# maraxen/trex

Measured on AMD Instinct MI355X. Metric: site-node-state updates/sec (Sankoff fwd+grad), higher is better.
Workload: dtype f32; 1 GPU; C4: 1024 random 32-taxa topologies x 5000 sites x 4 states, softmin tau=0.5 fwd (DP table written) + grad, split over 1 GPU(s) (1024 trees on rank 0); trees=1024, trees_rank0=1024, taxa=32, sites=5000, states=4, hipgraph=True, parallelism=tree-batch x1, settle_steps=35

## Files before the change

trex_amd/csrc/plan.cpp:

```cpp
#include <algorithm>
#include <cstdlib>
#include <cstdint>
#include <cstring>
#include <functional>
#include <queue>
#include <set>
#include <vector>

#include "trex_common.h"

namespace trex {

namespace {

constexpr int kKindSent = 0, kKindLeaf = 1, kKindInt = 2;

struct Child {
  int kind;
  int index;
};

bool plan_one_tree(const int32_t* ch, int n_all, int32_t* fwd, int32_t* bt,
                   int* n_slots, int* bt_ok, int* n_dag, int* n_unreached) {
  const int nl = (n_all + 1) / 2;
  const int ni = n_all - nl;
  std::vector<Child> kids(2 * ni);
  std::vector<int> refs(ni, 0);
  for (int r = 0; r < ni; ++r) {
    const int node = nl + r;
    for (int k = 0; k < 2; ++k) {
      const int c = ch[2 * node + k];
      if (c < -1 || c >= n_all) return false;
      Child cd;
      if (c == -1 || c >= node) {
        cd = {kKindSent, 0};
      } else if (c < nl) {
        cd = {kKindLeaf, c};
      } else {
        cd = {kKindInt, c - nl};
        refs[c - nl] += 1;
      }
      kids[2 * r + k] = cd;
    }
  }
  int dag = 0;
  for (int r = 0; r < ni; ++r) dag += refs[r] > 1;
  *n_dag = dag;

  std::vector<int> need(ni, 1);
  for (int r = 0; r < ni; ++r) {
    int a = 0, b = 0;
    for (int k = 0; k < 2; ++k) {
      const Child& cd = kids[2 * r + k];
      if (cd.kind == kKindInt) {
        const int n = need[cd.index];
        if (n > a) { b = a; a = n; } else if (n > b) { b = n; }
      }
    }
    need[r] = std::max({1, a, b + 1});
  }

  std::vector<int> order;
  order.reserve(ni);
  std::vector<char> done(ni, 0);
  auto visit = [&](int start) {
    std::vector<std::pair<int, int>> st;
    st.push_back({start, 0});
    while (!st.empty()) {
      auto [r, ph] = st.back();
      st.pop_back();
      if (done[r]) continue;
      if (ph == 1) {
        done[r] = 1;
        order.push_back(r);
        continue;
// ... 7 lines not shown
      if (light >= 0 && !done[light]) st.push_back({light, 0});
      if (heavy >= 0 && !done[heavy]) st.push_back({heavy, 0});
    }
  };
  for (int r = 0; r < ni - 1; ++r)
    if (refs[r] == 0) visit(r);
  visit(ni - 1);
  if ((int)order.size() != ni) return false;

  std::vector<int> pos(ni, 0), consumer(ni, -1);
  for (int k = 0; k < ni; ++k) pos[order[k]] = k;
  for (int r = 0; r < ni; ++r)
    for (int k = 0; k < 2; ++k)
      if (kids[2 * r + k].kind == kKindInt) consumer[kids[2 * r + k].index] = r;
  std::vector<char> bypass(ni, 0);
  for (int r = 0; r < ni; ++r)
    bypass[r] = refs[r] == 1 && consumer[r] >= 0 && pos[consumer[r]] == pos[r] + 1;

  std::vector<int> remaining(refs), slot(ni, 0xFF);
  std::set<int> free_slots;
  int top = 0, maxs = 0;
  for (int r : order) {
    for (int k = 0; k < 2; ++k) {
      const Child& cd = kids[2 * r + k];
      if (cd.kind != kKindInt || bypass[cd.index]) continue;
      if (--remaining[cd.index] == 0) free_slots.insert(slot[cd.index]);
    }
    if (refs[r] > 0 && !bypass[r]) {
      int s;
      if (!free_slots.empty()) {
        s = *free_slots.begin();
        free_slots.erase(free_slots.begin());
      } else {
        s = top++;
      }
      slot[r] = s;
      maxs = std::max(maxs, s + 1);
    }
  }
  if (maxs > 250) return false;
  *n_slots = maxs;

  std::vector<char> reach(ni, 0);
  reach[ni - 1] = 1;
  for (int r = ni - 1; r >= 0; --r) {
    if (!reach[r]) continue;
    for (int k = 0; k < 2; ++k)
      if (kids[2 * r + k].kind == kKindInt) reach[kids[2 * r + k].index] = 1;
  }
  int unr = 0;
  for (int r = 0; r < ni; ++r) unr += !reach[r];
  *n_unreached = unr;

  static const bool defer_on = [] {
    const char* e = std::getenv("TREX_DEFER");
    return !(e && e[0] == '0');
  }();
  std::vector<char> deferred(ni, 0);
  if (defer_on)
    for (int c = 0; c < ni; ++c)
      deferred[c] = refs[c] == 1 && consumer[c] >= 0 && reach[consumer[c]] &&
                    kids[2 * c].kind != kKindInt && kids[2 * c + 1].kind != kKindInt;

  std::vector<char> seen(ni, 0);
  std::vector<int32_t> enc(4 * ni);
  for (int k = ni - 1; k >= 0; --k) {
    const int r = order[k];
    int32_t* e = &enc[4 * k];
    e[0] = (r & 0xFFFF) | ((slot[r] & 0xFF) << 16);
    for (int j = 0; j < 2; ++j) {
      const Child& cd = kids[2 * r + j];
      int32_t d = (cd.index & 0xFFFF) | (cd.kind << 24);
      if (cd.kind == kKindInt) {
        d |= (slot[cd.index] & 0xFF) << 16;
        if (bypass[cd.index]) d |= kChildPrev;
        if (deferred[cd.index]) d |= kChildDeferred;
        if (reach[r]) {
          if (seen[cd.index]) d |= kStepAccumulate;
          seen[cd.index] = 1;
        }
      }
      e[1 + j] = d;
    }
    int32_t f = 0;
    if (r == ni - 1) f |= kStepRoot;
    if (!reach[r]) f |= kStepUnreached;
    if (bypass[r]) f |= kStepToNext;
    if (deferred[r]) f |= kStepDeferredIn;
    e[3] = f;
  }
  if (order.back() != ni - 1) return false;
  std::memcpy(fwd, enc.data(), enc.size() * sizeof(int32_t));

  std::vector<int> last_parent(ni, -1), last_slot(ni, -1);
  std::vector<char> visited(ni, 0);
  std::vector<std::pair<int, int>> stk;
  stk.push_back({n_all - 1, -1});
  int64_t steps = 0;
  const int64_t cap = 1LL << 22;
  bool ok = true;
  while (!stk.empty()) {
    if (++steps > cap || (int64_t)stk.size() > 4LL * n_all) { ok = false; break; }
    auto [node, from] = stk.back();
    stk.pop_back();
    if (node < nl) continue;
    const int x = node - nl;
    visited[x] = 1;
    if (from >= 0) { last_parent[x] = from >> 1; last_slot[x] = from & 1; }
    const int c0 = ch[2 * node], c1 = ch[2 * node + 1];
    if (c0 == node || c1 == node) { ok = false; break; }
// ... 166 lines not shown
    if (kd == kKindSent) return 0;
    if (kd == kKindLeaf) return (c & 0xFFFF) | (kKindLeaf << 24);
    if (task[c]) return (c & 0xFFFF) | (slot[c] << 16) | (kKindInt << 24);
    const int32_t d0 = desc(c, 0), d1 = desc(c, 1);
    inl[c] = (int)(ient.size() / 4);
    ient.insert(ient.end(), {c, d0, d1, height[c]});
    return (inl[c] & 0xFFFF) | (kKindInline << 24);
  };
  const int n_steps = (int)order.size();
  int32_t* offs = region + 4;
  int32_t* steps = region + lp_steps_offset(ni);
  for (int s = 0; s <= S; ++s) offs[s] = n_steps;
  for (int k = n_steps - 1; k >= 0; --k) offs[stage[order[k]]] = k;
  for (int s = S - 1; s >= 0; --s) offs[s] = std::min(offs[s], offs[s + 1]);
  for (int k = 0; k < n_steps; ++k) {
    const int r = order[k];
    steps[4 * k] = (r & 0xFFFF) | (slot[r] << 16);
    steps[4 * k + 1] = desc(r, 0);
    steps[4 * k + 2] = desc(r, 1);
    steps[4 * k + 3] = r == root ? kStepRoot : 0;
  }
  if (!ient.empty()) std::memcpy(steps + 4LL * n_steps, ient.data(), ient.size() * sizeof(int32_t));
  region[0] = S;
  region[1] = n_slots;
  region[2] = n_steps;
  region[3] = (int)(ient.size() / 4);
  return n_slots;
}

}

}

extern "C" int64_t trex_plan_ints(int B, int n_all) {
  if (B <= 0 || n_all < 2) return 0;
  const int ni = n_all - (n_all + 1) / 2;
  return TREX_PLAN_HEADER_INTS + (int64_t)B * ni * 6 +
         (int64_t)B * (trex::staged_tree_ints(ni) + trex::lp_tree_ints(ni));
}

extern "C" int trex_plan_build(const int32_t* children, int B, int n_all,
                               int32_t* plan, int32_t* info) {
  using namespace trex;
  if (!children || !plan || B <= 0 || n_all < 3 || n_all > 65535)
    return set_error(TREX_E_ARG, "trex_plan_build: bad arguments (B=%d n_all=%d)", B, n_all);
  const int nl = (n_all + 1) / 2;
  const int ni = n_all - nl;
  std::memset(plan, 0, sizeof(int32_t) * TREX_PLAN_HEADER_INTS);
  int32_t* fwd = plan + TREX_PLAN_HEADER_INTS;
  int32_t* bt = fwd + (int64_t)B * ni * 4;
  int32_t* staged = bt + (int64_t)B * ni * 2;
  int32_t* lanes = staged + (int64_t)B * staged_tree_ints(ni);
  int max_slots = 0, all_bt_ok = 1, dag = 0, unr = 0, lp_slots = 0;
  for (int b = 0; b < B; ++b) {
    int s = 0, ok = 0, d = 0, u = 0;
    if (!plan_one_tree(children + (int64_t)b * n_all * 2, n_all, fwd + (int64_t)b * ni * 4,
                       bt + (int64_t)b * ni * 2, &s, &ok, &d, &u))
      return set_error(TREX_E_TOPOLOGY, "trex_plan_build: tree %d has an invalid child list", b);
    stage_one_tree(children + (int64_t)b * n_all * 2, n_all, staged + b * staged_tree_ints(ni));
    const int ls = lane_program_one_tree(children + (int64_t)b * n_all * 2, n_all,
                                         lanes + b * lp_tree_ints(ni));
    lp_slots = (ls < 0 || lp_slots < 0) ? -1 : std::max(lp_slots, ls);
    max_slots = std::max(max_slots, s);
    all_bt_ok &= ok;
    dag += d;
    unr += u;
  }
  plan[0] = kPlanMagic;
  plan[1] = B;
  plan[2] = n_all;
  plan[3] = nl;
  plan[4] = ni;
  plan[5] = max_slots;
  plan[6] = all_bt_ok;
  plan[7] = lp_slots;
  if (info) {
    info[0] = max_slots | ((lp_slots < 0 ? 0 : lp_slots + 1) << 16);
    info[1] = all_bt_ok;
    info[2] = dag;
    info[3] = unr;
  }
  return TREX_OK;
}

namespace trex {
namespace {
constexpr int32_t kRaggedMagic = 0x54525247;
constexpr int kRaggedMetaInts = 12;

bool ragged_shapes(const int32_t* n_all, const int32_t* L, int B, int64_t* steps, int64_t* items) {
  *steps = 0;
  *items = 0;
  for (int b = 0; b < B; ++b) {
    if (n_all[b] < 3 || n_all[b] > 65535 || L[b] <= 0) return false;
    *steps += n_all[b] - (n_all[b] + 1) / 2;
    *items += (L[b] + 63) / 64;
  }
  return *items <= 0x7FFFFFFF;
}
}
}

extern "C" int64_t trex_ragged_plan_ints(int B, const int32_t* n_all, const int32_t* L) {
  if (B <= 0 || !n_all || !L) return 0;
  int64_t steps, items;
  if (!trex::ragged_shapes(n_all, L, B, &steps, &items)) return 0;
  return TREX_PLAN_HEADER_INTS + (int64_t)B * trex::kRaggedMetaInts + items + steps * 6;
}

extern "C" int trex_ragged_plan_build(const int32_t* children, const int32_t* n_all,
                                      const int32_t* L, int B, int32_t* plan, int64_t* info) {
  using namespace trex;
  int64_t steps, items;
  if (!children || !n_all || !L || !plan || B <= 0 || !ragged_shapes(n_all, L, B, &steps, &items))
    return set_error(TREX_E_ARG, "trex_ragged_plan_build: bad arguments (B=%d)", B);
  int32_t* meta = plan + TREX_PLAN_HEADER_INTS;
  int32_t* ritem = meta + (int64_t)B * kRaggedMetaInts;
  int32_t* fwd = ritem + items;
  int32_t* bt = fwd + steps * 4;
  std::memset(plan, 0, sizeof(int32_t) * TREX_PLAN_HEADER_INTS);
  int64_t step_off = 0, item_off = 0, site_off = 0, leaf_off = 0, rows_off = 0, child_off = 0;
  int max_slots = 0, max_nl = 0, max_ni = 0, all_ok = 1, dag = 0, unr = 0;
  for (int b = 0; b < B; ++b) {
    const int na = n_all[b];
    const int nl = (na + 1) / 2;
    const int ni = na - nl;
    int s = 0, ok = 0, d = 0, u = 0;
    if (!plan_one_tree(children + child_off, na, fwd + step_off * 4, bt + step_off * 2, &s, &ok, &d,
                       &u))
      return set_error(TREX_E_TOPOLOGY, "trex_ragged_plan_build: tree %d has an invalid child list",
                       b);
    if (site_off > 0x7FFFFFFF)
      return set_error(TREX_E_UNSUPPORTED, "trex_ragged_plan_build: more than 2^31 sites");
    if ((int64_t)ni * L[b] * 4 * 4 > 0x7FFFFFF0LL)
      return set_error(TREX_E_UNSUPPORTED, "trex_ragged_plan_build: tree %d's DP table exceeds 2 GiB",
                       b);
    int32_t* m = meta + (int64_t)b * kRaggedMetaInts;
    m[0] = (int32_t)step_off;
    m[1] = ni;
    m[2] = nl;
    m[3] = L[b];
    m[4] = (int32_t)site_off;
    m[5] = (int32_t)item_off;
    m[6] = (int32_t)(leaf_off & 0xFFFFFFFF);
    m[7] = (int32_t)(leaf_off >> 32);
    m[8] = (int32_t)(rows_off & 0xFFFFFFFF);
    m[9] = (int32_t)(rows_off >> 32);
    const int tiles = (L[b] + 63) / 64;
    for (int t = 0; t < tiles; ++t) ritem[item_off + t] = b;
    max_slots = std::max(max_slots, s);
    max_nl = std::max(max_nl, nl);
    max_ni = std::max(max_ni, ni);
    all_ok &= ok;
    dag += d;
    unr += u;
    step_off += ni;
    item_off += tiles;
    site_off += L[b];
    leaf_off += (int64_t)nl * L[b];
    rows_off += (int64_t)ni * L[b];
    child_off += 2LL * na;
  }
  plan[0] = kRaggedMagic;
  plan[1] = B;
  plan[2] = (int32_t)steps;
  plan[3] = (int32_t)items;
  plan[4] = max_slots;
  plan[5] = max_nl;
  plan[6] = all_ok;
  plan[7] = max_ni;
  if (info) {
    info[0] = max_slots;
    info[1] = max_nl;
    info[2] = items;
    info[3] = leaf_off;
    info[4] = rows_off;
    info[5] = site_off;
    info[6] = all_ok;
    info[7] = dag + ((int64_t)unr << 32);
  }
  return TREX_OK;
}
// ... 1 lines not shown
```

trex_amd/csrc/sankoff.hip:

```cpp
#include <hip/hip_runtime.h>

#include <algorithm>
#include <cmath>
#include <cstdlib>
#include <cstring>
#include <mutex>
#include <string>

#include "sankoff_dev.h"
#include "trex_common.h"

namespace trex {

namespace {

thread_local char g_err[512] = "no error";


template <int SPT>
__device__ __forceinline__ void ld(const float* __restrict__ p, float (&o)[SPT]) {
  if constexpr (SPT == 4) {
    const float4 v = *reinterpret_cast<const float4*>(p);
    o[0] = v.x; o[1] = v.y; o[2] = v.z; o[3] = v.w;
  } else if constexpr (SPT == 2) {
// ... 301 lines not shown
    for (int i = 0; i < Q; ++i) sv[i] = kdot<Q>(cf.k[i], u);
  }
}

template <int Q, int SPT, int MODE, bool SYM = false>
__device__ __forceinline__ void message(const Coef<Q>& cf, float a, float bcoef,
                                        const float (&d)[Q][SPT], float (&m)[Q][SPT]) {
  if constexpr (MODE == kHard) {
#pragma unroll
    for (int i = 0; i < Q; ++i)
#pragma unroll
      for (int s = 0; s < SPT; ++s) {
        float v = cf.c[i][0] + d[0][s];
#pragma unroll
        for (int j = 1; j < Q; ++j) v = fminf(v, cf.c[i][j] + d[j][s]);
        m[i][s] = v;
      }
  } else if constexpr (MODE == kSoftK) {
#pragma unroll
    for (int s = 0; s < SPT; ++s) {
      float md = d[0][s];
#pragma unroll
      for (int j = 1; j < Q; ++j) md = fminf(md, d[j][s]);
      const float mda = md * a;
      float u[Q];
#pragma unroll
      for (int j = 0; j < Q; ++j) u[j] = fast_exp2(fmaf(-d[j][s], a, mda));
      const float base = md + cf.cmin;
      float sv[Q];
      kvec<Q, SYM>(cf, u, sv);
#pragma unroll
      for (int i = 0; i < Q; ++i) m[i][s] = fmaf(-bcoef, fast_log2(sv[i]), base);
    }
  } else {
#pragma unroll
    for (int i = 0; i < Q; ++i)
#pragma unroll
      for (int s = 0; s < SPT; ++s) {
        float x[Q];
        float mn = INFINITY;
#pragma unroll
        for (int j = 0; j < Q; ++j) {
          x[j] = cf.c[i][j] + d[j][s];
          mn = fminf(mn, x[j]);
        }
        float acc = 0.0f;
#pragma unroll
        for (int j = 0; j < Q; ++j) acc += fast_exp2((mn - x[j]) * a);
        m[i][s] = fmaf(-bcoef, fast_log2(acc), mn);
      }
  }
}

template <int Q, int SPT, int MODE, bool SYM = false>
__device__ __forceinline__ void message_adjoint(const Coef<Q>& cf, float a,
                                                const float (&d)[Q][SPT],
                                                const float (&g)[Q][SPT],
                                                float (&acc)[Q][Q], float (&gc)[Q][SPT]) {
#pragma unroll
  for (int s = 0; s < SPT; ++s) {
    if constexpr (MODE == kHard) {
#pragma unroll
      for (int j = 0; j < Q; ++j) gc[j][s] = 0.0f;
#pragma unroll
      for (int i = 0; i < Q; ++i) {
        float x[Q];
        float mn = cf.c[i][0] + d[0][s];
        x[0] = mn;
#pragma unroll
        for (int j = 1; j < Q; ++j) {
          x[j] = cf.c[i][j] + d[j][s];
          mn = fminf(mn, x[j]);
        }
        float cnt = 0.0f;
#pragma unroll
        for (int j = 0; j < Q; ++j) cnt += (x[j] == mn) ? 1.0f : 0.0f;
        const float r = g[i][s] / cnt;
#pragma unroll
        for (int j = 0; j < Q; ++j) {
          const float w = (x[j] == mn) ? r : 0.0f;
          acc[i][j] += w;
          gc[j][s] += w;
        }
      }
    } else if constexpr (MODE == kSoftK) {
      float md = d[0][s];
#pragma unroll
      for (int j = 1; j < Q; ++j) md = fminf(md, d[j][s]);
      const float mda = md * a;
      float u[Q];
#pragma unroll
      for (int j = 0; j < Q; ++j) u[j] = fast_exp2(fmaf(-d[j][s], a, mda));
      float r[Q];
      float sv[Q];
      kvec<Q, SYM>(cf, u, sv);
#pragma unroll
      for (int i = 0; i < Q; ++i) r[i] = g[i][s] * __builtin_amdgcn_rcpf(sv[i]);
#pragma unroll
      for (int i = 0; i < Q; ++i) axpy<Q>(acc[i], r[i], u);
      float t[Q];
#pragma unroll
      for (int j = 0; j < Q; ++j) t[j] = r[0] * cf.k[0][j];
#pragma unroll
      for (int i = 1; i < Q; ++i) axpy<Q>(t, r[i], cf.k[i]);
#pragma unroll
      for (int j = 0; j < Q; ++j) gc[j][s] = u[j] * t[j];
    } else {
#pragma unroll
      for (int j = 0; j < Q; ++j) gc[j][s] = 0.0f;
#pragma unroll
      for (int i = 0; i < Q; ++i) {
        float x[Q];
        float mn = INFINITY;
#pragma unroll
        for (int j = 0; j < Q; ++j) {
          x[j] = cf.c[i][j] + d[j][s];
          mn = fminf(mn, x[j]);
        }
        float e[Q];
        float sm = 0.0f;
#pragma unroll
        for (int j = 0; j < Q; ++j) {
          e[j] = fast_exp2((mn - x[j]) * a);
          sm += e[j];
        }
        const float r = g[i][s] * __builtin_amdgcn_rcpf(sm);
#pragma unroll
        for (int j = 0; j < Q; ++j) {
          const float w = r * e[j];
          acc[i][j] += w;
          gc[j][s] += w;
        }
      }
    }
  }
}

template <int Q, int SPT, bool SOFT>
__device__ __forceinline__ void root_score(const float (&d)[Q][SPT], float a, float bcoef,
                                           bool hard_root, float (&score)[SPT],
                                           float (&w)[Q][SPT]) {
#pragma unroll
  for (int s = 0; s < SPT; ++s) {
    float mn = d[0][s];
#pragma unroll
    for (int i = 1; i < Q; ++i) mn = fminf(mn, d[i][s]);
    if (!SOFT || hard_root) {
      float cnt = 0.0f;
#pragma unroll
      for (int i = 0; i < Q; ++i) cnt += (d[i][s] == mn) ? 1.0f : 0.0f;
      const float r = 1.0f / cnt;
#pragma unroll
      for (int i = 0; i < Q; ++i) w[i][s] = (d[i][s] == mn) ? r : 0.0f;
      score[s] = mn;
    } else {
      float sm = 0.0f;
#pragma unroll
      for (int i = 0; i < Q; ++i) {
        w[i][s] = fast_exp2((mn - d[i][s]) * a);
        sm += w[i][s];
      }
      const float r = __builtin_amdgcn_rcpf(sm);
#pragma unroll
      for (int i = 0; i < Q; ++i) w[i][s] *= r;
      score[s] = fmaf(-bcoef, fast_log2(sm), mn);
    }
  }
}


struct KArgs {
  const int4* steps;
  const int8_t* leaves;
  const float* cost;
  int n_int, nl, L, tiles, B, n_slots;
  float a, bcoef;
  int hard_root;
  float* dp;
  float* site_score;
  float* tree_score;
  const float* dts;
  float* marg;
  int8_t* anc;
  float* d_cost;
  double* part_tree;
  double* part_dc;
  int nblocks;
  const int* rmeta;
  const int* ritem;
};



constexpr int kTabFloats = 128;
constexpr int kWTab = 32;
#ifndef TREX_ADJ_RING
#define TREX_ADJ_RING 3
#endif
#ifndef TREX_ADJ_WPE
#define TREX_ADJ_WPE 5
#endif
#ifndef TREX_FUSED_WPE
#define TREX_FUSED_WPE TREX_ADJ_WPE
#endif
#ifndef TREX_FUSED_WPE_MAX
#define TREX_FUSED_WPE_MAX 8
#endif
#ifndef TREX_FWD_WPE
#define TREX_FWD_WPE 6
#endif
constexpr int kAdjRing = TREX_ADJ_RING;
constexpr int kPrefetchRows = 64;

template <int Q, int SPT, int MODE, int PHASE, bool RAGGED, bool SYM = false>
__device__ __forceinline__ void sankoff_body(const KArgs& A, float* lds) {
  static_assert(!RAGGED || SPT == 1, "ragged batches use the SPT=1 kernels");
  constexpr bool SOFT = MODE != kHard;
  constexpr bool FWD = (PHASE & 1) != 0;
  constexpr bool BWD = (PHASE & 2) != 0;
  const int lane = threadIdx.x;
  const int L = A.L;
  const float a = A.a, bcoef = A.bcoef;
  const int nb = A.nblocks;
  const int per = (nb + 7) / 8;
  const int xcd = blockIdx.x & 7;
  const int stride = gridDim.x >> 3;
  const int item_end = min(nb, (xcd + 1) * per);
  int item = xcd * per + (blockIdx.x >> 3);
  if (item >= item_end) return;

  Coef<Q> cf;
  load_coef<Q, MODE>(A.cost, a, cf);

  float* tab = lds;
  float* slots = lds + kTabFloats;
  constexpr int kRootSlot = 0;
  int8_t* lleaf = reinterpret_cast<int8_t*>(slots + (size_t)max(A.n_slots, 1) * Q * kWave * SPT);

  {
    float cmn, cmx;
    cost_range<Q>(A.cost, cmn, cmx);
    const float range = cmx - cmn;
    const bool lfast = (MODE != kHard) ? ((kSentinel - range) * a >= 64.0f) : (range < 99000.0f);
    if (lane <= Q) {
      const cptr<float> cost = as_const(A.cost);
      float d1[Q][1], m1[Q][1], g1[Q][1], w1[Q][Q], gc1[Q][1];
#pragma unroll
      for (int j = 0; j < Q; ++j) {
        d1[j][0] = j == lane ? 0.0f : kSentinel;
        g1[j][0] = 1.0f;
      }
#pragma unroll
      for (int i = 0; i < Q; ++i)
#pragma unroll
        for (int j = 0; j < Q; ++j) w1[i][j] = 0.0f;
      if (lfast && lane < Q) {
#pragma unroll
        for (int i = 0; i < Q; ++i) {
          const float cv = cost[i * Q + lane];
          m1[i][0] = cv;
          const float ik = MODE == kSoftK ? fast_exp2((cv - cf.cmin) * a) : 1.0f;
#pragma unroll
          for (int j = 0; j < Q; ++j) w1[i][j] = j == lane ? ik : 0.0f;
        }
      } else {
        message<Q, 1, MODE>(cf, a, bcoef, d1, m1);
        message_adjoint<Q, 1, MODE>(cf, a, d1, g1, w1, gc1);
      }
#pragma unroll
      for (int i = 0; i < Q; ++i) {
        tab[lane * Q + i] = m1[i][0];
#pragma unroll
        for (int j = 0; j < Q; ++j) tab[kWTab + (lane * Q + i) * Q + j] = w1[i][j];
      }
    }
  }

  constexpr bool PERSIST = PHASE == 1;
  const bool pf = !RAGGED && SPT == 1 && (L & 3) == 0 && A.nl <= kPrefetchRows;
  const int pf_voff = (lane >> 4) * L + (lane & 15) * 4;
  uint32_t pre[kPrefetchRows / 4];
  auto issue_prefetch = [&](int it) {
    const int tr = it / A.tiles;
    const int tl = it - tr * A.tiles;
    const rsrc_t rl = make_rsrc(A.leaves + (size_t)tr * A.nl * L, (uint32_t)((size_t)A.nl * L));
#pragma unroll
    for (int r = 0; r < kPrefetchRows / 4; ++r)
      pre[r] = __builtin_amdgcn_raw_buffer_load_b32(rl, pf_voff, 4 * r * L + tl * kWave, TREX_AUX_LEAF);
  };
  auto store_prefetch = [&]() {
    uint32_t* dst = reinterpret_cast<uint32_t*>(lleaf);
#pragma unroll
    for (int r = 0; r < kPrefetchRows / 4; ++r) {
      const int row = 4 * r + (lane >> 4);
      if (row < A.nl) dst[row * 16 + (lane & 15)] = pre[r];
    }
  };
  if (pf) issue_prefetch(item);
  __syncthreads();

  do {
    int tree, tile, n_int, nl, Lt;
    size_t leaf_base, rows_base, site_base;
    cptr<int> prog;
    if constexpr (RAGGED) {
      tree = as_const(A.ritem)[item];
      const cptr<int> m = as_const(A.rmeta) + (size_t)tree * kRaggedMeta;
      n_int = m[1];
      nl = m[2];
      Lt = m[3];
      site_base = (size_t)(uint32_t)m[4];
      tile = item - m[5];
      leaf_base = (size_t)(uint32_t)m[6] | ((size_t)(uint32_t)m[7] << 32);
      rows_base = (size_t)(uint32_t)m[8] | ((size_t)(uint32_t)m[9] << 32);
      prog = as_const(reinterpret_cast<const int*>(A.steps)) + (size_t)m[0] * 4;
    } else {
      tree = item / A.tiles;
      tile = item - tree * A.tiles;
      n_int = A.n_int;
      nl = A.nl;
      Lt = L;
      leaf_base = (size_t)tree * A.nl * L;
      rows_base = (size_t)tree * A.n_int * L;
      site_base = (size_t)tree * L;
      prog = as_const(reinterpret_cast<const int*>(A.steps)) + (size_t)tree * A.n_int * 4;
    }
    const int site = (tile * kWave + lane) * SPT;
    const bool active = site < Lt;
    const int sc = active ? site : 0;

    if (pf) {
      store_prefetch();
      if (PERSIST && item + stride < item_end) issue_prefetch(item + stride);
    } else {
      const int8_t* lv = A.leaves + leaf_base + sc;
      constexpr int kBatch = 8;
      for (int c0 = 0; c0 < nl; c0 += kBatch) {
        int code[kBatch][SPT];
        const int nb_ = min(kBatch, nl - c0);
#pragma unroll
        for (int u = 0; u < kBatch; ++u)
          if (u < nb_) ld_codes<SPT>(lv + (size_t)(c0 + u) * Lt, code[u]);
#pragma unroll
        for (int u = 0; u < kBatch; ++u)
          if (u < nb_) st_codes<SPT>(lleaf + ((c0 + u) * kWave + lane) * SPT, code[u]);
      }
    }

    const uint32_t treebytes = (uint32_t)((size_t)n_int * Q * Lt * 4);
    const rsrc_t rdp = make_rsrc(A.dp + rows_base * Q, treebytes);
    const int voff = active ? site * Q * 4 : 0x7FFFFFF0;
    const int rowbytes = Lt * Q * 4;

    auto child_code = [&](int desc, int (&code)[SPT]) {
      ld_codes<SPT>(lleaf + ((desc & 0xFFFF) * kWave + lane) * SPT, code);
#pragma unroll
      for (int s = 0; s < SPT; ++s) code[s] = ((unsigned)code[s] < (unsigned)Q) ? code[s] : Q;
    };

    float dv[Q][SPT];
    if constexpr (FWD) {
      float prev[Q][SPT];
      I4 nxt = load_step(prog, 0);
      for (int k = 0; k < n_int; ++k) {
        const I4 stp = nxt;
        if (k + 1 < n_int) nxt = load_step(prog, k + 1);
        float d[2][Q][SPT];
#pragma unroll
        for (int c = 0; c < 2; ++c) {
          const int desc = c == 0 ? stp.y : stp.z;
          const int kind = (desc >> 24) & 3;
          if (desc & kChildPrev) {
#pragma unroll
            for (int j = 0; j < Q; ++j)
#pragma unroll
              for (int s = 0; s < SPT; ++s) d[c][j][s] = prev[j][s];
          } else if (kind == kKindInt) {
            lds_get<Q, SPT>(slots, (desc >> 16) & 0xFF, lane, d[c]);
          } else {
            int code[SPT];
            if (kind == kKindLeaf) {
              child_code(desc, code);
            } else {
#pragma unroll
              for (int s = 0; s < SPT; ++s) code[s] = Q;
            }
#pragma unroll
            for (int s = 0; s < SPT; ++s) {
              float r[Q];
              lds_vec_get<Q>(tab + code[s] * Q, r);
#pragma unroll
              for (int i = 0; i < Q; ++i) d[c][i][s] = r[i];
            }
          }
        }
#pragma unroll
        for (int c = 0; c < 2; ++c) {
          const int desc = c == 0 ? stp.y : stp.z;
          float m[Q][SPT];
          if (((desc >> 24) & 3) != kKindInt) {
#pragma unroll
            for (int i = 0; i < Q; ++i)
#pragma unroll
              for (int s = 0; s < SPT; ++s) m[i][s] = d[c][i][s];
          } else {
            message<Q, SPT, MODE, false>(cf, a, bcoef, d[c], m);
          }
#pragma unroll
          for (int i = 0; i < Q; ++i)
#pragma unroll
            for (int s = 0; s < SPT; ++s) dv[i][s] = (c == 0) ? m[i][s] : dv[i][s] + m[i][s];
        }
        const int row = stp.x & 0xFFFF;
        const int oslot = (stp.x >> 16) & 0xFF;
#ifdef TREX_DIAG_PAD
        diag_pad(dv[0][0]);
#endif
#ifdef TREX_DIAG_NOSTORE
        bst_row<Q, SPT, BWD ? kAuxFusedRow : kAuxFwdRow>(rdp, 0x7FFFFFF0, row * rowbytes, dv);
#elif defined(TREX_DIAG_DROP)
        const bool drop = TREX_DIAG_DROP > 0 ? k < TREX_DIAG_DROP : k >= n_int + TREX_DIAG_DROP;
        bst_row<Q, SPT, BWD ? kAuxFusedRow : kAuxFwdRow>(rdp, drop ? 0x7FFFFFF0 : voff,
                                                        row * rowbytes, dv);
#else
        if (BWD && kAuxCherryRow != kAuxFusedRow && (stp.w & kStepDeferredIn))
          bst_row<Q, SPT, kAuxCherryRow>(rdp, voff, row * rowbytes, dv);
        else
          bst_row<Q, SPT, BWD ? kAuxFusedRow : kAuxFwdRow>(rdp, voff, row * rowbytes, dv);
#endif
        if (!(stp.w & kStepToNext) && oslot != 0xFF) {
          lds_put<Q, SPT>(slots, oslot, lane, dv);
        }
#pragma unroll
        for (int i = 0; i < Q; ++i)
#pragma unroll
          for (int s = 0; s < SPT; ++s) prev[i][s] = dv[i][s];
      }
    } else {
      bld_row<Q, SPT>(rdp, voff, (n_int - 1) * rowbytes, dv);
    }

    float score[SPT], groot[Q][SPT];
    root_score<Q, SPT, SOFT>(dv, a, bcoef, A.hard_root != 0, score, groot);
    if constexpr (FWD) {
      double tot = 0.0;
      if (active) {
#pragma unroll
        for (int s = 0; s < SPT; ++s) tot += (double)score[s];
        if (A.site_score) st<SPT>(A.site_score + site_base + site, score);
      }
      tot = wave_sum_lane0(tot);
      if (lane == 0) A.part_tree[item] = tot;
    }

    if constexpr (BWD) {
      float acc[Q][Q];
      const float dscale = A.dts ? as_const(A.dts)[tree] : 1.0f;
      const float f = active ? dscale : 0.0f;
#pragma unroll
      for (int i = 0; i < Q; ++i)
#pragma unroll
        for (int s = 0; s < SPT; ++s) groot[i][s] *= f;
#pragma unroll
      for (int i = 0; i < Q; ++i)
#pragma unroll
        for (int j = 0; j < Q; ++j) acc[i][j] = 0.0f;
      const bool want_marg = A.marg != nullptr;
      const rsrc_t rmg = make_rsrc(want_marg ? A.marg + rows_base * Q : A.dp, treebytes);
      int8_t* at = A.anc ? A.anc + rows_base + sc : nullptr;
      lds_put<Q, SPT>(slots, kRootSlot, lane, groot);

      auto prefetch = [&](const I4& s2, float (&nd)[2][Q][SPT]) {
#pragma unroll
        for (int c = 0; c < 2; ++c) {
          const int desc = c == 0 ? s2.y : s2.z;
          const bool internal =
              ((desc >> 24) & 3) == kKindInt && !(desc & kChildDeferred);
#ifdef TREX_DIAG_NOLOAD
          const int vo = 0x7FFFFFF0 + 0 * (internal ? voff : 0);
#else
          const int vo = internal ? voff : 0x7FFFFFF0;
#endif
          const int crow = internal ? (desc & 0xFFFF) : 0;
          bld_row<Q, SPT, FWD ? kAuxFusedLoad : kAuxAdjRow>(rdp, vo, crow * rowbytes, nd[c]);
        }
      };
      float gnext[Q][SPT];
      auto bstep = [&](const I4& stp, float (&cd)[2][Q][SPT]) {
        if (stp.w & kStepUnreached) return;
        const int row = stp.x & 0xFFFF;
#ifdef TREX_DIAG_PAD
        diag_pad(acc[0][0]);
#endif
        float g[Q][SPT];
        if (stp.w & kStepToNext) {
#pragma unroll
          for (int i = 0; i < Q; ++i)
#pragma unroll
            for (int s = 0; s < SPT; ++s) g[i][s] = gnext[i][s];
        } else {
          lds_get<Q, SPT>(slots, (stp.w & kStepRoot) ? kRootSlot : ((stp.x >> 16) & 0xFF), lane, g);
        }
        auto leaf_codes = [&](int desc, int kind, int (&code)[SPT]) {
          if (kind == kKindLeaf) {
            child_code(desc, code);
          } else {
#pragma unroll
            for (int s = 0; s < SPT; ++s) code[s] = Q;
          }
        };
        if (stp.w & kStepDeferredIn) {
          float dc[Q][SPT];
#pragma unroll
          for (int c = 0; c < 2; ++c) {
            const int desc = c == 0 ? stp.y : stp.z;
            int code[SPT];
            leaf_codes(desc, (desc >> 24) & 3, code);
#pragma unroll
            for (int s = 0; s < SPT; ++s) {
              float r[Q];
              lds_vec_get<Q>(tab + code[s] * Q, r);
#pragma unroll
              for (int i = 0; i < Q; ++i) dc[i][s] = (c == 0) ? r[i] : dc[i][s] + r[i];
            }
          }
          float gc[Q][SPT];
          message_adjoint<Q, SPT, MODE, SYM>(cf, a, dc, g, acc, gc);
#pragma unroll
          for (int i = 0; i < Q; ++i)
#pragma unroll
            for (int s = 0; s < SPT; ++s) g[i][s] = gc[i][s];
        }
        if (want_marg) {
          bst_row<Q, SPT, kAuxMarg>(rmg, voff, row * rowbytes, g);
        }
        if (at && active) {
          int best[SPT];
#pragma unroll
          for (int s = 0; s < SPT; ++s) {
            float bv = g[0][s];
            int bi = 0;
#pragma unroll
            for (int i = 1; i < Q; ++i)
              if (g[i][s] > bv) { bv = g[i][s]; bi = i; }
            best[s] = bi;
          }
          st_codes<SPT>(at + (size_t)row * Lt, best);
        }
#pragma unroll
        for (int c = 0; c < 2; ++c) {
          const int desc = c == 0 ? stp.y : stp.z;
          const int kind = (desc >> 24) & 3;
          if (kind != kKindInt) {
            int code[SPT];
            leaf_codes(desc, kind, code);
#pragma unroll
            for (int s = 0; s < SPT; ++s) {
              float w[Q * Q];
              lds_vec_get<Q * Q>(tab + kWTab + code[s] * Q * Q, w);
#pragma unroll
              for (int i = 0; i < Q; ++i) {
                float wr[Q];
#pragma unroll
                for (int j = 0; j < Q; ++j) wr[j] = w[i * Q + j];
                axpy<Q>(acc[i], g[i][s], wr);
              }
            }
          } else {
            float gc[Q][SPT];
            if (desc & kChildDeferred) {
#pragma unroll
              for (int j = 0; j < Q; ++j)
#pragma unroll
                for (int s = 0; s < SPT; ++s) gc[j][s] = g[j][s];
            } else {
              message_adjoint<Q, SPT, MODE, SYM>(cf, a, cd[c], g, acc, gc);
            }
            if (desc & kChildPrev) {
#pragma unroll
              for (int j = 0; j < Q; ++j)
// ... 178 lines not shown
          }
          out[s] = bi;
        }
      }
    }
    st_codes<SPT>(at + (size_t)x * L, out);
  }
}

__global__ __launch_bounds__(256) void to_trex_layout_kernel(const float* __restrict__ dp,
                                                            const int8_t* __restrict__ leaves,
                                                            int B, int L, int n_all, int nl, int Q,
                                                            float* __restrict__ out) {
  const size_t total = (size_t)B * n_all * L;
  const int ni = n_all - nl;
  for (size_t t = (size_t)blockIdx.x * blockDim.x + threadIdx.x; t < total;
       t += (size_t)gridDim.x * blockDim.x) {
    const int l = (int)(t % L);
    const size_t rest = t / L;
    const int node = (int)(rest % n_all);
    const int b = (int)(rest / n_all);
    float* o = out + (((size_t)b * L + l) * n_all + node) * Q;
    if (node < nl) {
      const int code = leaves[((size_t)b * nl + node) * L + l];
      for (int q = 0; q < Q; ++q) o[q] = (code == q) ? 0.0f : kSentinel;
    } else {
      const float* src = dp + (((size_t)b * ni + (node - nl)) * L + l) * Q;
      for (int q = 0; q < Q; ++q) o[q] = src[q];
    }
  }
}

struct Shape {
  int B, L, n_all, nl, ni, Q;
};

int check_shape(const char* fn, int B, int L, int n_all, int Q, Shape* sh) {
  if (B <= 0 || L <= 0 || n_all < 3 || n_all > 65535 || Q < 2)
    return set_error(TREX_E_ARG, "%s: bad shape B=%d L=%d n_all=%d Q=%d", fn, B, L, n_all, Q);
  if (Q > kBigMaxQ)
    return set_error(TREX_E_UNSUPPORTED, "%s: Q=%d > %d not supported by this build (int8 leaf "
                     "codes / ancestral states)", fn, Q, kBigMaxQ);
  sh->B = B;
  sh->L = L;
  sh->n_all = n_all;
  sh->nl = (n_all + 1) / 2;
  sh->ni = n_all - sh->nl;
  sh->Q = Q;
  return TREX_OK;
}

int tiles_for(int L, int spt) { return (L + kWave * spt - 1) / (kWave * spt); }

size_t lds_bytes(int n_slots, int nl, int Q, int spt) {
  const size_t b = (size_t)kTabFloats * 4 + (size_t)std::max(n_slots, 1) * Q * kWave * spt * 4 +
                   (size_t)nl * kWave * spt;
  return (b + 15) & ~(size_t)15;
}

constexpr size_t kLdsPerCu = 160 * 1024;

int device_cus() {
  static const int cus = [] {
    int dev = 0, n = 0;
    (void)hipGetDevice(&dev);
    if (hipDeviceGetAttribute(&n, hipDeviceAttributeMultiprocessorCount, dev) != hipSuccess || n <= 0)
      n = 256;
    return n;
  }();
  return cus;
}

int hip_check(const char* fn) {
  const hipError_t e = hipGetLastError();
  if (e != hipSuccess) return set_error(TREX_E_HIP, "%s: %s", fn, hipGetErrorString(e));
  return TREX_OK;
}

int64_t counters_bytes(int B) { return ((int64_t)4 * (B + 1) + 255) / 256 * 256; }

void tau_coefs(float tau, float* a, float* bcoef) {
  if (tau > 0.0f) {
    *a = (float)(1.4426950408889634 / (double)tau);
    *bcoef = (float)((double)tau * 0.6931471805599453);
  } else {
    *a = 0.0f;
    *bcoef = 0.0f;
  }
}

template <class K>
int persistent_grid(K kernel, size_t lds, int nitems) {
  static std::mutex mu;
  static int cus = 0;
  struct Entry { const void* k; size_t lds; int occ; };
  static Entry cache[64];
  static int ncache = 0;
  int occ = 0;
  {
    std::lock_guard<std::mutex> g(mu);
    if (cus == 0) {
      int dev = 0;
      (void)hipGetDevice(&dev);
      if (hipDeviceGetAttribute(&cus, hipDeviceAttributeMultiprocessorCount, dev) != hipSuccess)
        cus = 256;
    }
    for (int i = 0; i < ncache; ++i)
      if (cache[i].k == (const void*)kernel && cache[i].lds == lds) occ = cache[i].occ;
    if (occ == 0) {
// ... 85 lines not shown
  n_slots &= 0xFFFF;
  if (n_slots > 250) return set_error(TREX_E_ARG, "%s: bad n_slots", fn);
  if (Q > 4 || wide_small_q(B, L, Q)) {
    WideCall c;
    c.phase = phase;
    c.soft = tau > 0.0f;
    c.steps = plan + TREX_PLAN_HEADER_INTS;
    c.leaves = leaves;
    c.cost = cost;
    c.B = B;
    c.L = L;
    c.nl = s.nl;
    c.ni = s.ni;
    c.Q = Q;
    c.n_slots = n_slots;
    tau_coefs(tau, &c.a, &c.bcoef);
    c.hard_root = (flags & TREX_FLAG_HARD_ROOT) ? 1 : 0;
    c.dp = dp;
    c.site_score = site_score;
    c.tree_score = tree_score;
    c.dts = dts;
    c.marg = marg;
    c.anc = anc;
    c.d_cost = d_cost;
    c.workspace = workspace;
    c.stream = stream;
    if (Q > kWideMaxQ) return bigq_run(fn, c);
    const int32_t* staged = plan + TREX_PLAN_HEADER_INTS + (int64_t)B * s.ni * 6;
    const int32_t* lanes = staged + (int64_t)B * staged_tree_ints(s.ni);
    if (site_eligible(c, lp_slots)) {
      char* tail = static_cast<char*>(workspace) + wide_workspace_bytes(B, L, Q);
      int* flag = reinterpret_cast<int*>(tail - 128);
      float* kg = reinterpret_cast<float*>(tail - 3456);
      c.site_flag = flag;
      c.site_kg = kg;
      if (phase == 3 && srow_room && site_srow_on())
        c.site_srow = reinterpret_cast<float*>(static_cast<char*>(workspace) +
                                               site_srow_offset(B, L, Q));
      if (int e = wide_run(fn, c, false)) return e;
      if (int e = site2_on(lp_slots, c.nl, c.ni) ? site2_run(fn, c, lanes, lp_slots, flag, kg)
                                                 : site_run(fn, c, lanes, lp_slots, flag, kg))
        return e;
      return partial_reduce(fn, static_cast<double*>(workspace),
                            static_cast<double*>(workspace) + (int64_t)B * wide_tiles(L, Q), B,
                            wide_tiles(L, Q), Q, phase, tree_score, d_cost, stream, nullptr, 0, 0,
                            1, flag, site_tiles(L));
    }
    if (use_staged(B, L, Q, s.ni, s.nl, phase)) return staged_run(fn, c, staged);
    return wide_run(fn, c);
  }
  if ((int64_t)s.ni * L * Q * 4 > 0x7FFFFFF0LL)
    return set_error(TREX_E_UNSUPPORTED, "%s: one tree's DP table exceeds 2 GiB", fn);
  const int tiles = tiles_for(L, 1);
  const size_t lds = lds_bytes(n_slots, s.nl, Q, 1);
  if (lds > 65536) return set_error(TREX_E_UNSUPPORTED, "%s: LDS stack too deep", fn);
  if ((int64_t)B * tiles > 0x7FFFFFFF) return set_error(TREX_E_ARG, "%s: grid too large", fn);
  KArgs A;
  A.rmeta = nullptr;
  A.ritem = nullptr;
  A.steps = reinterpret_cast<const int4*>(plan + TREX_PLAN_HEADER_INTS);
  A.leaves = leaves;
  A.cost = cost;
  A.n_int = s.ni;
  A.nl = s.nl;
  A.L = L;
  A.tiles = tiles;
  A.B = B;
  A.n_slots = n_slots;
  tau_coefs(tau, &A.a, &A.bcoef);
  A.hard_root = (flags & TREX_FLAG_HARD_ROOT) ? 1 : 0;
  A.dp = dp;
  A.site_score = site_score;
  A.tree_score = tree_score;
  A.dts = dts;
  A.marg = marg;
  A.anc = anc;
  A.d_cost = d_cost;
  char* w = static_cast<char*>(workspace) + counters_bytes(B);
  A.part_tree = reinterpret_cast<double*>(w);
  A.nblocks = B * tiles;
  A.part_dc = A.part_tree + A.nblocks;
  const bool soft = tau > 0.0f;
  hipStream_t st = (hipStream_t)stream;
  switch (Q) {
    case 2: dispatch_q<2>(phase, soft, lds, st, A); break;
    case 3: dispatch_q<3>(phase, soft, lds, st, A); break;
    case 4: dispatch_q<4>(phase, soft, lds, st, A); break;
  }
  if (int e = hip_check(fn)) return e;
  return partial_reduce(fn, A.part_tree, A.part_dc, B, tiles, Q, phase, tree_score, d_cost, stream);
}

template <int Q, bool SOFT>
void launch_ragged(int phase, size_t lds, hipStream_t st, const KArgs& A) {
  auto go = [&](auto kernel) {
    const int grid = phase == 1 ? persistent_grid(kernel, lds, A.nblocks) : (A.nblocks + 7) / 8 * 8;
    hipLaunchKernelGGL(kernel, dim3(grid), dim3(kWave), lds, st, A);
  };
  if (phase == 1)
    go(sankoff_kernel<Q, 1, SOFT, 1, true>);
  else if (phase == 2)
    go(sankoff_kernel<Q, 1, SOFT, 2, true>);
  else
    go(sankoff_kernel<Q, 1, SOFT, 3, true>);
}

}
// ... 102 lines not shown

extern "C" int trex_sankoff_ragged(int phase, const int32_t* plan, int B, int n_slots, int max_nl,
                                   int64_t items, const int8_t* leaves, const float* cost, int Q,
                                   float tau, unsigned flags, float* dp, float* site_score,
                                   float* tree_score, const float* d_tree_score, float* d_cost,
                                   float* marginals, int8_t* anc_states, void* workspace,
                                   int64_t workspace_bytes, void* stream) {
  const char* fn = "trex_sankoff_ragged";
  if (phase < 1 || phase > 3) return set_error(TREX_E_ARG, "%s: phase must be 1, 2 or 3", fn);
  if (B <= 0 || items <= 0 || items > 0x7FFFFFFF || max_nl < 2 || Q < 2)
    return set_error(TREX_E_ARG, "%s: bad shape B=%d items=%lld max_nl=%d Q=%d", fn, B,
                     (long long)items, max_nl, Q);
  if (Q > kBigMaxQ)
    return set_error(TREX_E_UNSUPPORTED, "%s: Q=%d > %d not supported by this build (int8 leaf "
                     "codes / ancestral states)", fn, Q, kBigMaxQ);
  if (!plan || !leaves || !cost || !workspace || !dp)
    return set_error(TREX_E_ARG, "%s: null pointer argument", fn);
  if ((phase & 1) && !tree_score) return set_error(TREX_E_ARG, "%s: tree_score is required", fn);
  if ((phase & 2) && !d_cost) return set_error(TREX_E_ARG, "%s: d_cost is required", fn);
  if (!nonneg_finite_f32(tau))
    return set_error(TREX_E_ARG, "%s: tau must be finite and >= 0 (got %g)", fn, tau);
  if (workspace_bytes < trex_ragged_workspace_bytes(items, Q))
    return set_error(TREX_E_ARG, "%s: workspace too small", fn);
  if (n_slots < 0 || n_slots > 250) return set_error(TREX_E_ARG, "%s: bad n_slots", fn);
  if (flags & ~TREX_FLAG_HARD_ROOT) return set_error(TREX_E_ARG, "%s: unknown flags 0x%x", fn, flags);
  if (Q > 4) {
    const int* meta = plan + TREX_PLAN_HEADER_INTS;
    WideCall c;
    c.phase = phase;
    c.soft = tau > 0.0f;
    c.steps = meta + (size_t)B * kRaggedMeta + items;
    c.leaves = leaves;
    c.cost = cost;
    c.B = B;
    c.L = 0;
    c.nl = max_nl;
    c.ni = max_nl - 1;
    c.Q = Q;
    c.n_slots = n_slots;
    tau_coefs(tau, &c.a, &c.bcoef);
    c.hard_root = (flags & TREX_FLAG_HARD_ROOT) ? 1 : 0;
    c.dp = dp;
    c.site_score = site_score;
    c.tree_score = tree_score;
    c.dts = d_tree_score;
    c.marg = marginals;
    c.anc = anc_states;
    c.d_cost = d_cost;
    c.workspace = workspace;
    c.stream = stream;
    if (Q > kWideMaxQ) return bigq_ragged_run(fn, c, meta, meta + (size_t)B * kRaggedMeta, items);
    return wide_ragged_run(fn, c, meta, meta + (size_t)B * kRaggedMeta, items);
  }
  const size_t lds = lds_bytes(n_slots, max_nl, Q, 1);
  if (lds > 65536) return set_error(TREX_E_UNSUPPORTED, "%s: LDS stack too deep", fn);
  KArgs A;
  const int* meta = plan + TREX_PLAN_HEADER_INTS;
  A.rmeta = meta;
  A.ritem = meta + (size_t)B * kRaggedMeta;
  A.steps = reinterpret_cast<const int4*>(A.ritem + items);
  A.leaves = leaves;
  A.cost = cost;
  A.n_int = 0;
  A.nl = max_nl;
  A.L = 0;
  A.tiles = 0;
  A.B = B;
  A.n_slots = n_slots;
  tau_coefs(tau, &A.a, &A.bcoef);
  A.hard_root = (flags & TREX_FLAG_HARD_ROOT) ? 1 : 0;
  A.dp = dp;
  A.site_score = site_score;
  A.tree_score = tree_score;
  A.dts = d_tree_score;
  A.marg = marginals;
  A.anc = anc_states;
  A.d_cost = d_cost;
  A.nblocks = (int)items;
  A.part_tree = reinterpret_cast<double*>(workspace);
  A.part_dc = A.part_tree + items;
  const bool soft = tau > 0.0f;
  hipStream_t st = (hipStream_t)stream;
  switch (Q) {
    case 2: soft ? launch_ragged<2, true>(phase, lds, st, A) : launch_ragged<2, false>(phase, lds, st, A); break;
    case 3: soft ? launch_ragged<3, true>(phase, lds, st, A) : launch_ragged<3, false>(phase, lds, st, A); break;
    case 4: soft ? launch_ragged<4, true>(phase, lds, st, A) : launch_ragged<4, false>(phase, lds, st, A); break;
  }
  if (int e = hip_check(fn)) return e;
  return partial_reduce(fn, A.part_tree, A.part_dc, B, 0, Q, phase, tree_score, d_cost, stream,
                        meta + 5, kRaggedMeta, (int)items);
}

extern "C" int trex_sankoff_ragged_backtrack(const int32_t* plan, int B, int64_t items,
                                             int64_t steps, int backtrack_ok, const float* cost,
                                             const float* dp, int Q, int8_t* anc_states,
                                             void* stream) {
  const char* fn = "trex_sankoff_ragged_backtrack";
  if (B <= 0 || items <= 0 || items > 0x7FFFFFFF || steps <= 0 || Q < 2)
    return set_error(TREX_E_ARG, "%s: bad arguments", fn);
  if (Q > kBigMaxQ)
    return set_error(TREX_E_UNSUPPORTED, "%s: Q=%d > %d not supported by this build", fn, Q,
                     kBigMaxQ);
  if (!backtrack_ok)
    return set_error(TREX_E_TOPOLOGY,
                     "%s: the reference backtrack does not terminate on this batch (cyclic child "
                     "references)", fn);
  if (!plan || !cost || !dp || !anc_states) return set_error(TREX_E_ARG, "%s: null pointer", fn);
// ... 16 lines not shown
```

Measured before the change: 707.7 billion site-node-state updates/s.

## Precompute leaf-pair message and adjoint tables in LDS for deferred cherries

Adds per-block LDS tables indexed by the pair of leaf state codes (5x5 combinations), holding the forward softmin message and the soft-K adjoint weights (u and reciprocal sums) for cherry nodes whose two children are both leaves. Deferred steps then read these tables instead of recomputing exp/log per site in both forward and backward passes. Also makes the TREX_DEFER env read non-static so it is re-evaluated per plan build, and skips weight-table writes in forward-only mode. The cost is extra LDS per block and a small table-build prologue, which can lower occupancy. This path only exercises the generic (non-wide/staged) kernel, which may not be the one the benchmark runs.

```diff
diff --git a/trex_amd/csrc/plan.cpp b/trex_amd/csrc/plan.cpp
--- a/trex_amd/csrc/plan.cpp
+++ b/trex_amd/csrc/plan.cpp
@@ -20,7 +20,12 @@
   int index;
 };
 
-bool plan_one_tree(const int32_t* ch, int n_all, int32_t* fwd, int32_t* bt,
+bool defer_enabled() {
+  const char* e = std::getenv("TREX_DEFER");
+  return !(e && e[0] == '0');
+}
+
+bool plan_one_tree(const int32_t* ch, int n_all, bool defer_on, int32_t* fwd, int32_t* bt,
                    int* n_slots, int* bt_ok, int* n_dag, int* n_unreached) {
   const int nl = (n_all + 1) / 2;
   const int ni = n_all - nl;
@@ -134,10 +139,6 @@
   for (int r = 0; r < ni; ++r) unr += !reach[r];
   *n_unreached = unr;
 
-  static const bool defer_on = [] {
-    const char* e = std::getenv("TREX_DEFER");
-    return !(e && e[0] == '0');
-  }();
   std::vector<char> deferred(ni, 0);
   if (defer_on)
     for (int c = 0; c < ni; ++c)
@@ -410,10 +411,11 @@
   int32_t* staged = bt + (int64_t)B * ni * 2;
   int32_t* lanes = staged + (int64_t)B * staged_tree_ints(ni);
   int max_slots = 0, all_bt_ok = 1, dag = 0, unr = 0, lp_slots = 0;
+  const bool defer_on = defer_enabled();
   for (int b = 0; b < B; ++b) {
     int s = 0, ok = 0, d = 0, u = 0;
-    if (!plan_one_tree(children + (int64_t)b * n_all * 2, n_all, fwd + (int64_t)b * ni * 4,
-                       bt + (int64_t)b * ni * 2, &s, &ok, &d, &u))
+    if (!plan_one_tree(children + (int64_t)b * n_all * 2, n_all, defer_on,
+                       fwd + (int64_t)b * ni * 4, bt + (int64_t)b * ni * 2, &s, &ok, &d, &u))
       return set_error(TREX_E_TOPOLOGY, "trex_plan_build: tree %d has an invalid child list", b);
     stage_one_tree(children + (int64_t)b * n_all * 2, n_all, staged + b * staged_tree_ints(ni));
     const int ls = lane_program_one_tree(children + (int64_t)b * n_all * 2, n_all,
@@ -479,13 +481,14 @@
   std::memset(plan, 0, sizeof(int32_t) * TREX_PLAN_HEADER_INTS);
   int64_t step_off = 0, item_off = 0, site_off = 0, leaf_off = 0, rows_off = 0, child_off = 0;
   int max_slots = 0, max_nl = 0, max_ni = 0, all_ok = 1, dag = 0, unr = 0;
+  const bool defer_on = defer_enabled();
   for (int b = 0; b < B; ++b) {
     const int na = n_all[b];
     const int nl = (na + 1) / 2;
     const int ni = na - nl;
     int s = 0, ok = 0, d = 0, u = 0;
-    if (!plan_one_tree(children + child_off, na, fwd + step_off * 4, bt + step_off * 2, &s, &ok, &d,
-                       &u))
+    if (!plan_one_tree(children + child_off, na, defer_on, fwd + step_off * 4, bt + step_off * 2,
+                       &s, &ok, &d, &u))
       return set_error(TREX_E_TOPOLOGY, "trex_ragged_plan_build: tree %d has an invalid child list",
                        b);
     if (site_off > 0x7FFFFFFF)
diff --git a/trex_amd/csrc/sankoff.hip b/trex_amd/csrc/sankoff.hip
--- a/trex_amd/csrc/sankoff.hip
+++ b/trex_amd/csrc/sankoff.hip
@@ -377,6 +377,39 @@
   }
 }
 
+template <int Q, bool SYM>
+__device__ __forceinline__ void softk_weights(const Coef<Q>& cf, float a, const float (&d)[Q],
+                                              float (&u)[Q], float (&rs)[Q]) {
+  float md = d[0];
+#pragma unroll
+  for (int j = 1; j < Q; ++j) md = fminf(md, d[j]);
+  const float mda = md * a;
+#pragma unroll
+  for (int j = 0; j < Q; ++j) u[j] = fast_exp2(fmaf(-d[j], a, mda));
+  float sv[Q];
+  kvec<Q, SYM>(cf, u, sv);
+#pragma unroll
+  for (int i = 0; i < Q; ++i) rs[i] = __builtin_amdgcn_rcpf(sv[i]);
+}
+
+template <int Q>
+__device__ __forceinline__ void softk_edge(const Coef<Q>& cf, const float (&u)[Q],
+                                           const float (&rs)[Q], const float (&g)[Q],
+                                           float (&acc)[Q][Q], float (&gc)[Q]) {
+  float r[Q];
+#pragma unroll
+  for (int i = 0; i < Q; ++i) r[i] = g[i] * rs[i];
+#pragma unroll
+  for (int i = 0; i < Q; ++i) axpy<Q>(acc[i], r[i], u);
+  float t[Q];
+#pragma unroll
+  for (int j = 0; j < Q; ++j) t[j] = r[0] * cf.k[0][j];
+#pragma unroll
+  for (int i = 1; i < Q; ++i) axpy<Q>(t, r[i], cf.k[i]);
+#pragma unroll
+  for (int j = 0; j < Q; ++j) gc[j] = u[j] * t[j];
+}
+
 template <int Q, int SPT, int MODE, bool SYM = false>
 __device__ __forceinline__ void message_adjoint(const Coef<Q>& cf, float a,
                                                 const float (&d)[Q][SPT],
@@ -409,27 +442,16 @@
         }
       }
     } else if constexpr (MODE == kSoftK) {
-      float md = d[0][s];
-#pragma unroll
-      for (int j = 1; j < Q; ++j) md = fminf(md, d[j][s]);
-      const float mda = md * a;
-      float u[Q];
-#pragma unroll
-      for (int j = 0; j < Q; ++j) u[j] = fast_exp2(fmaf(-d[j][s], a, mda));
-      float r[Q];
-      float sv[Q];
-      kvec<Q, SYM>(cf, u, sv);
-#pragma unroll
-      for (int i = 0; i < Q; ++i) r[i] = g[i][s] * __builtin_amdgcn_rcpf(sv[i]);
-#pragma unroll
-      for (int i = 0; i < Q; ++i) axpy<Q>(acc[i], r[i], u);
-      float t[Q];
-#pragma unroll
-      for (int j = 0; j < Q; ++j) t[j] = r[0] * cf.k[0][j];
-#pragma unroll
-      for (int i = 1; i < Q; ++i) axpy<Q>(t, r[i], cf.k[i]);
-#pragma unroll
-      for (int j = 0; j < Q; ++j) gc[j][s] = u[j] * t[j];
+      float ds[Q], gs[Q], u[Q], rs[Q], gcs[Q];
+#pragma unroll
+      for (int j = 0; j < Q; ++j) {
+        ds[j] = d[j][s];
+        gs[j] = g[j][s];
+      }
+      softk_weights<Q, SYM>(cf, a, ds, u, rs);
+      softk_edge<Q>(cf, u, rs, gs, acc, gcs);
+#pragma unroll
+      for (int j = 0; j < Q; ++j) gc[j][s] = gcs[j];
     } else {
 #pragma unroll
       for (int j = 0; j < Q; ++j) gc[j][s] = 0.0f;
@@ -517,8 +539,17 @@
 
 
 
-constexpr int kTabFloats = 128;
+#ifndef TREX_PAIR_TABLES
+#define TREX_PAIR_TABLES 1
+#endif
+constexpr bool kPairTables = TREX_PAIR_TABLES != 0;
+constexpr int kLeafTabFloats = 128;
 constexpr int kWTab = 32;
+constexpr int kPairFloats = 100;
+constexpr int kPairFwd = 28;
+constexpr int tab_floats(int phase) {
+  return kLeafTabFloats + ((kPairTables && phase != 1) ? 3 * kPairFloats : 0);
+}
 #ifndef TREX_ADJ_RING
 #define TREX_ADJ_RING 3
 #endif
@@ -558,7 +589,11 @@
   load_coef<Q, MODE>(A.cost, a, cf);
 
   float* tab = lds;
-  float* slots = lds + kTabFloats;
+  float* slots = lds + tab_floats(PHASE);
+  float* tm = tab + (PHASE == 1 ? kPairFwd : kLeafTabFloats);
+  float* tu = tab + kLeafTabFloats + kPairFloats;
+  float* tr = tab + kLeafTabFloats + 2 * kPairFloats;
+  constexpr bool PAIR_ADJ = kPairTables && BWD && MODE == kSoftK;
   constexpr int kRootSlot = 0;
   int8_t* lleaf = reinterpret_cast<int8_t*>(slots + (size_t)max(A.n_slots, 1) * Q * kWave * SPT);
 
@@ -590,13 +625,41 @@
         }
       } else {
         message<Q, 1, MODE>(cf, a, bcoef, d1, m1);
-        message_adjoint<Q, 1, MODE>(cf, a, d1, g1, w1, gc1);
+        if constexpr (BWD) message_adjoint<Q, 1, MODE>(cf, a, d1, g1, w1, gc1);
       }
 #pragma unroll
       for (int i = 0; i < Q; ++i) {
         tab[lane * Q + i] = m1[i][0];
-#pragma unroll
-        for (int j = 0; j < Q; ++j) tab[kWTab + (lane * Q + i) * Q + j] = w1[i][j];
+        if constexpr (BWD) {
+#pragma unroll
+          for (int j = 0; j < Q; ++j) tab[kWTab + (lane * Q + i) * Q + j] = w1[i][j];
+        }
+      }
+    }
+  }
+  if constexpr (kPairTables) {
+    __syncthreads();
+    if (lane < (Q + 1) * (Q + 1)) {
+      const int c0 = lane / (Q + 1), c1 = lane - c0 * (Q + 1);
+      float t0[Q], t1[Q], d1[Q][1];
+      lds_vec_get<Q>(tab + c0 * Q, t0);
+      lds_vec_get<Q>(tab + c1 * Q, t1);
+#pragma unroll
+      for (int j = 0; j < Q; ++j) d1[j][0] = t0[j] + t1[j];
+      if constexpr (FWD) {
+        float m1[Q][1], mv[Q];
+        message<Q, 1, MODE, false>(cf, a, bcoef, d1, m1);
+#pragma unroll
+        for (int i = 0; i < Q; ++i) mv[i] = m1[i][0];
+        lds_vec_put<Q>(tm + lane * Q, mv);
+      }
+      if constexpr (PAIR_ADJ) {
+        float ds[Q], u[Q], rs[Q];
+#pragma unroll
+        for (int j = 0; j < Q; ++j) ds[j] = d1[j][0];
+        softk_weights<Q, SYM>(cf, a, ds, u, rs);
+        lds_vec_put<Q>(tu + lane * Q, u);
+        lds_vec_put<Q>(tr + lane * Q, rs);
       }
     }
   }
@@ -691,6 +754,9 @@
         const I4 stp = nxt;
         if (k + 1 < n_int) nxt = load_step(prog, k + 1);
         float d[2][Q][SPT];
+        int pair[SPT];
+#pragma unroll
+        for (int s = 0; s < SPT; ++s) pair[s] = 0;
 #pragma unroll
         for (int c = 0; c < 2; ++c) {
           const int desc = c == 0 ? stp.y : stp.z;
@@ -716,6 +782,7 @@
               lds_vec_get<Q>(tab + code[s] * Q, r);
 #pragma unroll
               for (int i = 0; i < Q; ++i) d[c][i][s] = r[i];
+              if constexpr (kPairTables) pair[s] = c == 0 ? code[s] * (Q + 1) : pair[s] + code[s];
             }
           }
         }
@@ -723,7 +790,7 @@
         for (int c = 0; c < 2; ++c) {
           const int desc = c == 0 ? stp.y : stp.z;
           float m[Q][SPT];
-          if (((desc >> 24) & 3) != kKindInt) {
+          if (((desc >> 24) & 3) != kKindInt || (kPairTables && (desc & kChildDeferred))) {
 #pragma unroll
             for (int i = 0; i < Q; ++i)
 #pragma unroll
@@ -753,6 +820,15 @@
         else
           bst_row<Q, SPT, BWD ? kAuxFusedRow : kAuxFwdRow>(rdp, voff, row * rowbytes, dv);
 #endif
+        if (kPairTables && (stp.w & kStepDeferredIn)) {
+#pragma unroll
+          for (int s = 0; s < SPT; ++s) {
+            float r[Q];
+            lds_vec_get<Q>(tm + pair[s] * Q, r);
+#pragma unroll
+            for (int i = 0; i < Q; ++i) dv[i][s] = r[i];
+          }
+        }
         if (!(stp.w & kStepToNext) && oslot != 0xFF) {
           lds_put<Q, SPT>(slots, oslot, lane, dv);
         }
@@ -835,22 +911,46 @@
           }
         };
         if (stp.w & kStepDeferredIn) {
-          float dc[Q][SPT];
-#pragma unroll
-          for (int c = 0; c < 2; ++c) {
-            const int desc = c == 0 ? stp.y : stp.z;
-            int code[SPT];
-            leaf_codes(desc, (desc >> 24) & 3, code);
+          float gc[Q][SPT];
+          if constexpr (PAIR_ADJ) {
+            int pair[SPT];
+#pragma unroll
+            for (int c = 0; c < 2; ++c) {
+              const int desc = c == 0 ? stp.y : stp.z;
+              int code[SPT];
+              leaf_codes(desc, (desc >> 24) & 3, code);
+#pragma unroll
+              for (int s = 0; s < SPT; ++s)
+                pair[s] = c == 0 ? code[s] * (Q + 1) : pair[s] + code[s];
+            }
 #pragma unroll
             for (int s = 0; s < SPT; ++s) {
-              float r[Q];
-              lds_vec_get<Q>(tab + code[s] * Q, r);
-#pragma unroll
-              for (int i = 0; i < Q; ++i) dc[i][s] = (c == 0) ? r[i] : dc[i][s] + r[i];
+              float u[Q], rs[Q], gs[Q], gcs[Q];
+              lds_vec_get<Q>(tu + pair[s] * Q, u);
+              lds_vec_get<Q>(tr + pair[s] * Q, rs);
+#pragma unroll
+              for (int i = 0; i < Q; ++i) gs[i] = g[i][s];
+              softk_edge<Q>(cf, u, rs, gs, acc, gcs);
+#pragma unroll
+              for (int j = 0; j < Q; ++j) gc[j][s] = gcs[j];
             }
+          } else {
+            float dc[Q][SPT];
+#pragma unroll
+            for (int c = 0; c < 2; ++c) {
+              const int desc = c == 0 ? stp.y : stp.z;
+              int code[SPT];
+              leaf_codes(desc, (desc >> 24) & 3, code);
+#pragma unroll
+              for (int s = 0; s < SPT; ++s) {
+                float r[Q];
+                lds_vec_get<Q>(tab + code[s] * Q, r);
+#pragma unroll
+                for (int i = 0; i < Q; ++i) dc[i][s] = (c == 0) ? r[i] : dc[i][s] + r[i];
+              }
+            }
+            message_adjoint<Q, SPT, MODE, SYM>(cf, a, dc, g, acc, gc);
           }
-          float gc[Q][SPT];
-          message_adjoint<Q, SPT, MODE, SYM>(cf, a, dc, g, acc, gc);
 #pragma unroll
           for (int i = 0; i < Q; ++i)
 #pragma unroll
@@ -1135,9 +1235,9 @@
 
 int tiles_for(int L, int spt) { return (L + kWave * spt - 1) / (kWave * spt); }
 
-size_t lds_bytes(int n_slots, int nl, int Q, int spt) {
-  const size_t b = (size_t)kTabFloats * 4 + (size_t)std::max(n_slots, 1) * Q * kWave * spt * 4 +
-                   (size_t)nl * kWave * spt;
+size_t lds_bytes(int n_slots, int nl, int Q, int spt, int phase) {
+  const size_t b = (size_t)tab_floats(phase) * 4 +
+                   (size_t)std::max(n_slots, 1) * Q * kWave * spt * 4 + (size_t)nl * kWave * spt;
   return (b + 15) & ~(size_t)15;
 }
 
@@ -1329,7 +1429,7 @@
   if ((int64_t)s.ni * L * Q * 4 > 0x7FFFFFF0LL)
     return set_error(TREX_E_UNSUPPORTED, "%s: one tree's DP table exceeds 2 GiB", fn);
   const int tiles = tiles_for(L, 1);
-  const size_t lds = lds_bytes(n_slots, s.nl, Q, 1);
+  const size_t lds = lds_bytes(n_slots, s.nl, Q, 1, phase);
   if (lds > 65536) return set_error(TREX_E_UNSUPPORTED, "%s: LDS stack too deep", fn);
   if ((int64_t)B * tiles > 0x7FFFFFFF) return set_error(TREX_E_ARG, "%s: grid too large", fn);
   KArgs A;
@@ -1538,7 +1638,7 @@
     if (Q > kWideMaxQ) return bigq_ragged_run(fn, c, meta, meta + (size_t)B * kRaggedMeta, items);
     return wide_ragged_run(fn, c, meta, meta + (size_t)B * kRaggedMeta, items);
   }
-  const size_t lds = lds_bytes(n_slots, max_nl, Q, 1);
+  const size_t lds = lds_bytes(n_slots, max_nl, Q, 1, phase);
   if (lds > 65536) return set_error(TREX_E_UNSUPPORTED, "%s: LDS stack too deep", fn);
   KArgs A;
   const int* meta = plan + TREX_PLAN_HEADER_INTS;
```

After: 733.6 billion site-node-state updates/s, median of 6. 1.04x the previous value.
